# aurianer/DLA-Future

Measured on AMD Instinct MI355X. Metric: fp64 Cholesky TFlop/s, higher is better.
Workload: dtype f64; 1 GPU; cholesky_d N=65536 nb=1024 uplo=L; grid=1x1, rank_order=column-major, transport=none, work_copies=5

## Files before the change

### dla_future_amd/csrc/device/mma_core.hpp

```cpp
#pragma once
#include "common.hpp"

namespace dlaf_mi355x {

template <class T, int BM_, int BN_, int WM_, int WN_, int BK_, bool PAIRED_ = false, int STAGES_ = 2,
          int THREADS_ = kThreads>
struct BlockCfg {
  using R = real_t<T>;
  static constexpr bool CX = TypeInfo<T>::is_complex;
  static constexpr int BM = BM_, BN = BN_, WM = WM_, WN = WN_, BK = BK_;
  static constexpr int THREADS = THREADS_, NWAVES = THREADS_ / 64;
  static constexpr int TM = WM / 16, TN = WN / 16;
  static constexpr int WAVES_M = BM / WM, WAVES_N = BN / WN;
  static_assert(WAVES_M * WAVES_N == NWAVES, "the wave tiles must cover the block");
  static_assert(BK % 4 == 0 && WM % 16 == 0 && WN % 16 == 0, "MFMA 16x16x4 granularity");
  static constexpr bool PAIRED = PAIRED_ && !CX;
  static constexpr bool CXI = PAIRED_ && CX;
  static_assert(!PAIRED || (TM % 2 == 0 && TN % 2 == 0), "paired rows: even tile counts");
  static constexpr int PAD = PAIRED_ ? 0 : kLdsPad;
  static constexpr int LDA = BM + PAD, LDB = BN + PAD;
  static constexpr int EPP = CX ? 64 : 1024 / (int) sizeof(T);
  static constexpr int PIECES_A = BK * BM / EPP, PIECES_B = BK * BN / EPP;
  static constexpr bool GLDS =
      (PAIRED && (EPP % BM == 0 || BM % EPP == 0) && (EPP % BN == 0 || BN % EPP == 0) && (BK * BM) % EPP == 0 &&
       (BK * BN) % EPP == 0 && PIECES_A % NWAVES == 0 && PIECES_B % NWAVES == 0) ||
      (CXI && sizeof(T) == 16 && BM % 64 == 0 && BN % 64 == 0 && PIECES_A % NWAVES == 0 && PIECES_B % NWAVES == 0);
  static constexpr int LPS = PIECES_A / NWAVES + PIECES_B / NWAVES;
  static constexpr int A_PLANE = BK * LDA, B_PLANE = BK * LDB;
  static constexpr int A_ELEMS = (CX ? 2 : 1) * A_PLANE, B_ELEMS = (CX ? 2 : 1) * B_PLANE;
  static constexpr int BUF_ELEMS = A_ELEMS + B_ELEMS;
  static constexpr int STAGES = STAGES_;
  static_assert(STAGES >= 2 && STAGES <= 6, "2..6 LDS stages");
  static constexpr int LDS_BYTES = STAGES * BUF_ELEMS * (int) sizeof(R);
};

template <class Cfg>
struct Acc {
  using R = typename Cfg::R;
  using acc_t = typename Mma<R>::acc_t;
  acc_t re[Cfg::TM][Cfg::TN];
  acc_t im[Cfg::CX ? Cfg::TM : 1][Cfg::CX ? Cfg::TN : 1];

  __device__ __forceinline__ void clear() {
#pragma unroll
    for (int i = 0; i < Cfg::TM; ++i)
#pragma unroll
      for (int j = 0; j < Cfg::TN; ++j) {
        re[i][j] = acc_t{0, 0, 0, 0};
        if constexpr (Cfg::CX)
          im[i][j] = acc_t{0, 0, 0, 0};
      }
  }
};

struct NoHook {
  __device__ __forceinline__ void operator()(int) const {}
};

template <class Cfg, bool NEG = false, class Hook = NoHook>
__device__ __forceinline__ void mma_slab(const typename Cfg::R* __restrict__ As,
                                         const typename Cfg::R* __restrict__ Bs, Acc<Cfg>& acc, int wm,
                                         int wn, int lane, Hook&& hook = Hook{}) {
  using R = typename Cfg::R;
  const int g = lane >> 4, c = lane & 15;
#pragma unroll
  for (int k4 = 0; k4 < Cfg::BK / 4; ++k4) {
    const int kk = k4 * 4 + g;
    R a_re[Cfg::TM], a_im[Cfg::TM], b_re[Cfg::TN], b_im[Cfg::TN];
    if constexpr (Cfg::CXI) {
      typedef R r2 __attribute__((ext_vector_type(2)));
#pragma unroll
      for (int i = 0; i < Cfg::TM; ++i) {
        const r2 v = *reinterpret_cast<const r2*>(&As[2 * (kk * Cfg::LDA + wm * Cfg::WM + i * 16 + c)]);
        a_re[i] = v[0];
        a_im[i] = v[1];
      }
#pragma unroll
      for (int j = 0; j < Cfg::TN; ++j) {
        const r2 v = *reinterpret_cast<const r2*>(&Bs[2 * (kk * Cfg::LDB + wn * Cfg::WN + j * 16 + c)]);
        b_re[j] = v[0];
        b_im[j] = v[1];
      }
    }
    else if constexpr (Cfg::PAIRED) {
      typedef R r2 __attribute__((ext_vector_type(2)));
#pragma unroll
      for (int q = 0; q < Cfg::TM / 2; ++q) {
        const r2 v = *reinterpret_cast<const r2*>(&As[kk * Cfg::LDA + wm * Cfg::WM + q * 32 + 2 * c]);
        a_re[2 * q] = v[0];
        a_re[2 * q + 1] = v[1];
      }
#pragma unroll
      for (int q = 0; q < Cfg::TN / 2; ++q) {
        const r2 v = *reinterpret_cast<const r2*>(&Bs[kk * Cfg::LDB + wn * Cfg::WN + q * 32 + 2 * c]);
        b_re[2 * q] = v[0];
        b_re[2 * q + 1] = v[1];
      }
    }
    else {
#pragma unroll
      for (int i = 0; i < Cfg::TM; ++i) {
        a_re[i] = As[kk * Cfg::LDA + wm * Cfg::WM + i * 16 + c];
        if constexpr (Cfg::CX)
          a_im[i] = As[Cfg::A_PLANE + kk * Cfg::LDA + wm * Cfg::WM + i * 16 + c];
      }
#pragma unroll
      for (int j = 0; j < Cfg::TN; ++j) {
        b_re[j] = Bs[kk * Cfg::LDB + wn * Cfg::WN + j * 16 + c];
        if constexpr (Cfg::CX)
          b_im[j] = Bs[Cfg::B_PLANE + kk * Cfg::LDB + wn * Cfg::WN + j * 16 + c];
      }
    }
#pragma unroll
    for (int j = 0; j < Cfg::TN; ++j) {
      hook(k4 * Cfg::TN + j);
#pragma unroll
      for (int i = 0; i < Cfg::TM; ++i) {
        if constexpr (!NEG) {
          acc.re[i][j] = Mma<R>::mma(b_re[j], a_re[i], acc.re[i][j]);
          if constexpr (Cfg::CX) {
            acc.re[i][j] = Mma<R>::mma(b_im[j], a_im[i], acc.re[i][j]);
            acc.im[i][j] = Mma<R>::mma(b_re[j], a_im[i], acc.im[i][j]);
            acc.im[i][j] = Mma<R>::mma_neg(b_im[j], a_re[i], acc.im[i][j]);
          }
        }
        else {
          acc.re[i][j] = Mma<R>::mma_neg(b_re[j], a_re[i], acc.re[i][j]);
          if constexpr (Cfg::CX) {
            acc.re[i][j] = Mma<R>::mma_neg(b_im[j], a_im[i], acc.re[i][j]);
            acc.im[i][j] = Mma<R>::mma_neg(b_re[j], a_im[i], acc.im[i][j]);
            acc.im[i][j] = Mma<R>::mma(b_im[j], a_re[i], acc.im[i][j]);
          }
        }
      }
    }
  }
}

template <class Cfg>
__device__ __forceinline__ int acc_m(int i, int c) {
  if constexpr (Cfg::PAIRED)
    return (i >> 1) * 32 + 2 * c + (i & 1);
  else
    return i * 16 + c;
}
template <class Cfg>
__device__ __forceinline__ int acc_n(int j, int g, int v) {
  using R = typename Cfg::R;
  if constexpr (Cfg::PAIRED)
    return (j >> 1) * 32 + 2 * Mma<R>::irow(g, v) + (j & 1);
  else
    return j * 16 + Mma<R>::irow(g, v);
}

template <class Cfg, class T>
__device__ __forceinline__ void stage_glds(const T* __restrict__ A, long lda, const T* __restrict__ B, long ldb, int k0,
                                           typename Cfg::R* __restrict__ buf, int wave, int lane) {
  constexpr int NA = Cfg::PIECES_A / Cfg::NWAVES, NB = Cfg::PIECES_B / Cfg::NWAVES;
  constexpr int QA0 = 0, QA1 = NA, QB0 = 0, QB1 = NB;
  if constexpr (Cfg::CXI) {
    constexpr int PA = Cfg::BM / 64, PB = Cfg::BN / 64;
#pragma unroll
    for (int idx = QA0; idx < QA1; ++idx) {
      const int piece = wave + Cfg::NWAVES * idx;
      const int k = piece / PA, part = piece % PA;
      const T* ga = A + part * 64 + lane + (long) (k0 + k) * lda;
      __builtin_amdgcn_global_load_lds((const __attribute__((address_space(1))) void*) ga,
                                       (__attribute__((address_space(3))) void*) (buf + 2 * (k * Cfg::LDA + part * 64)),
                                       16, 0, 0);
    }
#pragma unroll
    for (int idx = QB0; idx < QB1; ++idx) {
      const int piece = wave + Cfg::NWAVES * idx;
      const int k = piece / PB, part = piece % PB;
      const T* gb = B + part * 64 + lane + (long) (k0 + k) * ldb;
      __builtin_amdgcn_global_load_lds(
          (const __attribute__((address_space(1))) void*) gb,
          (__attribute__((address_space(3))) void*) (buf + Cfg::A_ELEMS + 2 * (k * Cfg::LDB + part * 64)), 16, 0, 0);
    }
    return;
  }
  constexpr int PER = 16 / (int) sizeof(T);
  constexpr int EPP = Cfg::EPP;
#pragma unroll
  for (int q = QA0; q < QA1; ++q) {
    const int e0 = (wave * NA + q) * EPP;
    const int e = e0 + lane * PER;
    const T* ga = A + (e % Cfg::BM) + (long) (k0 + e / Cfg::BM) * lda;
    __builtin_amdgcn_global_load_lds((const __attribute__((address_space(1))) void*) ga,
                                     (__attribute__((address_space(3))) void*) (buf + e0), 16, 0, 0);
  }
#pragma unroll
  for (int q = QB0; q < QB1; ++q) {
    const int e0 = (wave * NB + q) * EPP;
    const int e = e0 + lane * PER;
    const T* gb = B + (e % Cfg::BN) + (long) (k0 + e / Cfg::BN) * ldb;
    __builtin_amdgcn_global_load_lds((const __attribute__((address_space(1))) void*) gb,
                                     (__attribute__((address_space(3))) void*) (buf + Cfg::A_ELEMS + e0), 16, 0, 0);
  }
}

template <class Cfg, class T, int IDX>
__device__ __forceinline__ void stage_glds_one(const T* __restrict__ A, long lda, const T* __restrict__ B, long ldb,
                                               int k0, typename Cfg::R* __restrict__ buf, int wave, int lane) {
  static_assert(!Cfg::CXI, "real types");
  constexpr int NA = Cfg::PIECES_A / Cfg::NWAVES, NB = Cfg::PIECES_B / Cfg::NWAVES;
  constexpr int PER = 16 / (int) sizeof(T), EPP = Cfg::EPP;
  auto at = [](const T* base, unsigned byte_off) {
    return reinterpret_cast<const T*>(reinterpret_cast<const char*>(base) + byte_off);
  };
  if constexpr (IDX < NA) {
    static_assert(EPP % Cfg::BM == 0 || Cfg::BM % EPP == 0, "pieces and columns nest");
    const int e0 = (wave * NA + IDX) * EPP;
    const unsigned loff = (unsigned) sizeof(T) * (unsigned) ((lane * PER) % Cfg::BM + ((lane * PER) / Cfg::BM) * (int) lda);
    const T* ga = A + (e0 % Cfg::BM) + (long) (k0 + e0 / Cfg::BM) * lda;
    __builtin_amdgcn_global_load_lds((const __attribute__((address_space(1))) void*) at(ga, loff),
                                     (__attribute__((address_space(3))) void*) (buf + e0), 16, 0, 0);
  }
  else if constexpr (IDX < NA + NB) {
    static_assert(EPP % Cfg::BN == 0 || Cfg::BN % EPP == 0, "pieces and columns nest");
    const int e0 = (wave * NB + (IDX - NA)) * EPP;
    const unsigned loff = (unsigned) sizeof(T) * (unsigned) ((lane * PER) % Cfg::BN + ((lane * PER) / Cfg::BN) * (int) ldb);
    const T* gb = B + (e0 % Cfg::BN) + (long) (k0 + e0 / Cfg::BN) * ldb;
    __builtin_amdgcn_global_load_lds((const __attribute__((address_space(1))) void*) at(gb, loff),
                                     (__attribute__((address_space(3))) void*) (buf + Cfg::A_ELEMS + e0), 16, 0, 0);
  }
}

template <class Cfg, class T, bool VEC, bool EDGE, bool UTAIL = false, bool NEG = false>
__device__ __forceinline__ void gemm_nt_block(const T* __restrict__ A, long lda, int mrows,
                                              const T* __restrict__ B, long ldb, int ncols, int K,
                                              typename Cfg::R* __restrict__ lds, Acc<Cfg>& acc, int K1 = 1 << 30,
                                              const T* __restrict__ A2 = nullptr,
                                              const T* __restrict__ B2 = nullptr, int s0 = 0) {
  using R = typename Cfg::R;
  const int lane = threadIdx.x & 63;
  const int wave = __builtin_amdgcn_readfirstlane(threadIdx.x >> 6);
  const int wm = wave % Cfg::WAVES_M, wn = wave / Cfg::WAVES_M;
  const int nk = (K + Cfg::BK - 1) / Cfg::BK;
  if (nk == 0)
    return;
  if constexpr (Cfg::GLDS && VEC && !EDGE) {
    constexpr int ST = Cfg::STAGES;
    constexpr int LPS = Cfg::LPS;
    static_assert(LPS * (ST - 2) < 64, "vmcnt is a 6-bit counter");
#pragma unroll
    for (int s = 0; s < ST - 1; ++s)
      if (s < nk) {
        int sl = s0 + s;
        sl = sl >= nk ? sl - nk : sl;
        stage_glds<Cfg, T>(sl * Cfg::BK < K1 ? A : A2, lda, sl * Cfg::BK < K1 ? B : B2, ldb, sl * Cfg::BK,
                           lds + s * Cfg::BUF_ELEMS, wave, lane);
      }
    if (nk >= ST - 1)
      __builtin_amdgcn_s_waitcnt(0x0070 | ((LPS * (ST - 2)) & 0xF) | ((((LPS * (ST - 2)) >> 4) & 0x3) << 14));
    else
      asm volatile("s_waitcnt vmcnt(0)" ::: "memory");
    __builtin_amdgcn_s_barrier();
    int cur_i = 0, nxt_i = ST - 1;
    constexpr bool SPLIT = !Cfg::CXI && LPS <= (Cfg::BK / 4) * Cfg::TN && LPS <= 16;
    for (int kt = 0; kt < nk; ++kt) {
      R* cur = lds + cur_i * Cfg::BUF_ELEMS;
      const bool load = UTAIL || (kt + ST - 1 < nk);
      int sn = s0 + min(kt + ST - 1, nk - 1);
      sn = sn >= nk ? sn - nk : sn;
      const int kn = sn * Cfg::BK;
      const T* An = kn < K1 ? A : A2;
      const T* Bn = kn < K1 ? B : B2;
      R* nbuf = lds + nxt_i * Cfg::BUF_ELEMS;
      if constexpr (SPLIT) {
        mma_slab<Cfg, NEG>(cur, cur + Cfg::A_ELEMS, acc, wm, wn, lane, [&](int p) {
#define DLAF_GLDS_AT(I)                                                                     \
  if (p == I) {                                                                           \
    if constexpr (I < LPS)                                                                \
      if (load)                                                                           \
        stage_glds_one<Cfg, T, (I < LPS ? I : 0)>(An, lda, Bn, ldb, kn, nbuf, wave, lane); \
  }
          DLAF_GLDS_AT(0) DLAF_GLDS_AT(1) DLAF_GLDS_AT(2) DLAF_GLDS_AT(3) DLAF_GLDS_AT(4) DLAF_GLDS_AT(5)
          DLAF_GLDS_AT(6) DLAF_GLDS_AT(7) DLAF_GLDS_AT(8) DLAF_GLDS_AT(9) DLAF_GLDS_AT(10) DLAF_GLDS_AT(11)
          DLAF_GLDS_AT(12) DLAF_GLDS_AT(13) DLAF_GLDS_AT(14) DLAF_GLDS_AT(15)
#undef DLAF_GLDS_AT
        });
      }
      else {
        if (load)
          stage_glds<Cfg, T>(An, lda, Bn, ldb, kn, nbuf, wave, lane);
        mma_slab<Cfg, NEG>(cur, cur + Cfg::A_ELEMS, acc, wm, wn, lane);
      }
      if (load)
        __builtin_amdgcn_s_waitcnt(0x0070 | ((LPS * (ST - 2)) & 0xF) | ((((LPS * (ST - 2)) >> 4) & 0x3) << 14));
      else
        asm volatile("s_waitcnt vmcnt(0)" ::: "memory");
      asm volatile("s_waitcnt lgkmcnt(0)" ::: "memory");
      __builtin_amdgcn_s_barrier();
      cur_i = (cur_i + 1 == ST) ? 0 : cur_i + 1;
      nxt_i = (nxt_i + 1 == ST) ? 0 : nxt_i + 1;
    }
    if constexpr (UTAIL) {
      asm volatile("s_waitcnt vmcnt(0)" ::: "memory");
      __builtin_amdgcn_s_barrier();
    }
    return;
  }
  Slab<T, Cfg::BM, Cfg::BK, VEC, Cfg::LDA, Cfg::CXI, Cfg::THREADS> sa;
  Slab<T, Cfg::BN, Cfg::BK, VEC, Cfg::LDB, Cfg::CXI, Cfg::THREADS> sb;
  sa.template load<EDGE>(0 < K1 ? A : A2, lda, 0, mrows, K, A2, K1);
  sb.template load<EDGE>(0 < K1 ? B : B2, ldb, 0, ncols, K, B2, K1);
  sa.store(lds);
  sb.store(lds + Cfg::A_ELEMS);
  __syncthreads();
  for (int kt = 0; kt < nk; ++kt) {
    R* cur = lds + (kt & 1) * Cfg::BUF_ELEMS;
    R* nxt = lds + ((kt + 1) & 1) * Cfg::BUF_ELEMS;
    const bool more = (kt + 1) < nk;
    if (more) {
      const int kn = (kt + 1) * Cfg::BK;
      sa.template load<EDGE>(kn < K1 ? A : A2, lda, kn, mrows, K, A2, K1);
      sb.template load<EDGE>(kn < K1 ? B : B2, ldb, kn, ncols, K, B2, K1);
    }
    mma_slab<Cfg, NEG>(cur, cur + Cfg::A_ELEMS, acc, wm, wn, lane);
    if (more) {
      sa.store(nxt);
      sb.store(nxt + Cfg::A_ELEMS);
    }
    __syncthreads();
  }
}

}
```

Before: 68.77 TFlop/s.

## Software-pipeline LDS reads with rotated quadrant MFMA schedule in fp64 slab

Adds a specialized fp64 paired 4x4-tile inner slab that issues ds_read_b128 loads asynchronously via inline asm, with explicit lgkmcnt waits. The MFMA work is split into quadrants so next-k loads overlap with current MFMAs. Sched barriers pin the order. This aims to hide LDS latency inside the GEMM/SYRK core, at the cost of fragile hand-scheduled asm and extra register pressure.

```diff
diff --git a/dla_future_amd/csrc/device/mma_core.hpp b/dla_future_amd/csrc/device/mma_core.hpp
--- a/dla_future_amd/csrc/device/mma_core.hpp
+++ b/dla_future_amd/csrc/device/mma_core.hpp
@@ -57,11 +57,105 @@
   __device__ __forceinline__ void operator()(int) const {}
 };
 
+typedef double lds_pair_d __attribute__((ext_vector_type(2)));
+
+template <int OFF>
+__device__ __forceinline__ void lds_read_pair_async(lds_pair_d& v, unsigned addr) {
+  static_assert(OFF >= 0 && OFF < 65536 && OFF % 16 == 0, "ds_read_b128: 16-bit unsigned offset, 16-byte aligned");
+  asm volatile("ds_read_b128 %0, %1 offset:%2" : "=v"(v) : "v"(addr), "i"(OFF) : "memory");
+}
+template <int N>
+__device__ __forceinline__ void lds_wait_pairs(lds_pair_d& x, lds_pair_d& y) {
+  asm volatile("s_waitcnt lgkmcnt(%2)" : "+v"(x), "+v"(y) : "i"(N) : "memory");
+}
+template <int N>
+__device__ __forceinline__ void lds_wait_pairs(lds_pair_d& x) {
+  asm volatile("s_waitcnt lgkmcnt(%1)" : "+v"(x) : "i"(N) : "memory");
+}
+
+template <class Cfg>
+inline constexpr bool kRotatedSlab = Cfg::PAIRED && Cfg::TM == 4 && Cfg::TN == 4 && sizeof(typename Cfg::R) == 8 &&
+                                     (Cfg::BK / 4) % 2 == 0;
+
+template <class Cfg, bool NEG>
+__device__ __forceinline__ void mma_quadrant(Acc<Cfg>& acc, int jp, int ip, const lds_pair_d& b, const lds_pair_d& a) {
+#pragma unroll
+  for (int jj = 0; jj < 2; ++jj)
+#pragma unroll
+    for (int ii = 0; ii < 2; ++ii) {
+      auto& d = acc.re[2 * ip + ii][2 * jp + jj];
+      if constexpr (!NEG)
+        d = Mma<double>::mma(b[jj], a[ii], d);
+      else
+        d = Mma<double>::mma_neg(b[jj], a[ii], d);
+    }
+}
+
+template <class Cfg, bool NEG, int K4, class Hook>
+__device__ __forceinline__ void mma_slab_rotated_step(unsigned a_addr, unsigned b_addr, Acc<Cfg>& acc, lds_pair_d (&a)[2],
+                                                      lds_pair_d& b0, lds_pair_d& b1, Hook& hook) {
+  constexpr int NS = Cfg::BK / 4;
+  constexpr bool NEXT = K4 + 1 < NS;
+  constexpr int F = K4 & 1, S = 1 - F;
+  constexpr int KN = NEXT ? K4 + 1 : 0;
+  constexpr int AOFF = 8 * (KN * 4 * Cfg::LDA), BOFF = 8 * (KN * 4 * Cfg::LDB);
+
+  hook(4 * K4 + 0);
+  lds_wait_pairs<2>(b0, a[F]);
+  mma_quadrant<Cfg, NEG>(acc, 0, F, b0, a[F]);
+  __builtin_amdgcn_sched_barrier(0);
+
+  hook(4 * K4 + 1);
+  lds_wait_pairs<1>(a[S]);
+  mma_quadrant<Cfg, NEG>(acc, 0, S, b0, a[S]);
+  if constexpr (NEXT)
+    lds_read_pair_async<BOFF>(b0, b_addr);
+  __builtin_amdgcn_sched_barrier(0);
+
+  hook(4 * K4 + 2);
+  lds_wait_pairs<NEXT ? 1 : 0>(b1);
+  mma_quadrant<Cfg, NEG>(acc, 1, S, b1, a[S]);
+  if constexpr (NEXT)
+    lds_read_pair_async<AOFF + 8 * 32 * S>(a[S], a_addr);
+  __builtin_amdgcn_sched_barrier(0);
+
+  hook(4 * K4 + 3);
+  mma_quadrant<Cfg, NEG>(acc, 1, F, b1, a[F]);
+  if constexpr (NEXT) {
+    lds_read_pair_async<AOFF + 8 * 32 * F>(a[F], a_addr);
+    lds_read_pair_async<BOFF + 8 * 32>(b1, b_addr);
+    __builtin_amdgcn_sched_barrier(0);
+    mma_slab_rotated_step<Cfg, NEG, K4 + 1>(a_addr, b_addr, acc, a, b0, b1, hook);
+  }
+}
+
+template <class Cfg, bool NEG, class Hook>
+__device__ __forceinline__ void mma_slab_rotated(const double* __restrict__ As, const double* __restrict__ Bs,
+                                                 Acc<Cfg>& acc, int wm, int wn, int lane, Hook& hook) {
+  static_assert(kRotatedSlab<Cfg> && Cfg::PAD == 0, "fp64, paired rows, 4 x 4 tiles, an even number of k-steps");
+  const int g = lane >> 4, c = lane & 15;
+  const unsigned a_addr = (unsigned) (uintptr_t) (const __attribute__((address_space(3))) double*) As +
+                          8u * (unsigned) (g * Cfg::LDA + wm * Cfg::WM + 2 * c);
+  const unsigned b_addr = (unsigned) (uintptr_t) (const __attribute__((address_space(3))) double*) Bs +
+                          8u * (unsigned) (g * Cfg::LDB + wn * Cfg::WN + 2 * c);
+  lds_pair_d a[2], b0, b1;
+  lds_read_pair_async<0>(b0, b_addr);
+  lds_read_pair_async<0>(a[0], a_addr);
+  lds_read_pair_async<8 * 32>(a[1], a_addr);
+  lds_read_pair_async<8 * 32>(b1, b_addr);
+  __builtin_amdgcn_sched_barrier(0);
+  mma_slab_rotated_step<Cfg, NEG, 0>(a_addr, b_addr, acc, a, b0, b1, hook);
+}
+
 template <class Cfg, bool NEG = false, class Hook = NoHook>
 __device__ __forceinline__ void mma_slab(const typename Cfg::R* __restrict__ As,
                                          const typename Cfg::R* __restrict__ Bs, Acc<Cfg>& acc, int wm,
                                          int wn, int lane, Hook&& hook = Hook{}) {
   using R = typename Cfg::R;
+  if constexpr (kRotatedSlab<Cfg>) {
+    mma_slab_rotated<Cfg, NEG>(As, Bs, acc, wm, wn, lane, hook);
+    return;
+  }
   const int g = lane >> 4, c = lane & 15;
 #pragma unroll
   for (int k4 = 0; k4 < Cfg::BK / 4; ++k4) {
```

Result: faster. 69.92 TFlop/s (median of 6 runs) (+1.7%).
